# zengxiaofei/HapHiC

Measured on AMD Instinct MI355X. Metric: Hi-C pairs/s ingested (link-matrix build) + MCL iters/s, higher is better.
Workload: dtype u64 keys + u32 counts (ingest); f32 values, exact u64 fixed-point accumulation (MCL)

## Files before the change

haphic_amd/csrc/hhx_expand.hip:

```cpp
#include <chrono>
#include <climits>

#include "hhx_common.h"
#include "hhx_internal.h"
#include "hhx_sort.h"

using namespace hhx;

struct ExpandDemand { i64 out = 0, cand = 0; };
thread_local ExpandDemand g_expand_hint, g_expand_demand;
void hhx_expand_set_hint(i64 out, i64 cand) { g_expand_hint.out = out; g_expand_hint.cand = cand; }
void hhx_expand_last_demand(i64 *out, i64 *cand) { *out = g_expand_demand.out; *cand = g_expand_demand.cand; }

namespace {

constexpr int EX_T_WIN = 1024;
constexpr int EX_T_CMP = 256;
constexpr int EX_T_MAX = 1024;
constexpr int EX_WAVES_MAX = EX_T_MAX / HHX_WAVE;
#define EX_T ((int)blockDim.x)
#define EX_WAVES ((int)blockDim.x / HHX_WAVE)
constexpr int STAGE = 1024;
constexpr int MAX_WIN = 512;
constexpr int N_DUMMY = HHX_WAVE;
// ... 1522 lines not shown
            const i32 len = min(STAGE, a_e - a0);
            stage_chunk(P, l, a0, len);
            __syncthreads();
            mark_compact(P, l, len);
            __syncthreads();
        }
        const i32 nnz_row = bitmap_prefix_total(l, W);
        nnzc += (tid == 0) ? nnz_row : 0;
        double s_run = 0.0;
        i32 n_win = 0;
        for (i32 r0 = 0; r0 < nnz_row; r0 += cap, ++n_win) {
            const i32 rlen = min(cap, nnz_row - r0);
            for (i32 t = tid; t < rlen; t += EX_T) l.acc[t] = 0;
            __syncthreads();
            for (i32 a0 = a_b; a0 < a_e; a0 += STAGE) {
                const i32 len = min(STAGE, a_e - a0);
                stage_chunk(P, l, a0, len);
                __syncthreads();
                accumulate_compact(P, l, len, r0, rlen);
                __syncthreads();
            }
            i32 nz;
            s_run += window_power_sum<true>(P, l, rlen, &nz);
            window_emit_candidates<true>(P, l, rlen, 0, r0, s_run, &l.win_off[n_win], &l.win_cnt[n_win]);
            __syncthreads();
        }
        if (nnz_row == 0) {
            if (tid == 0) { P.row_off[row] = 0; P.row_cnt[row] = 0; }
        } else finalize_row(P, l, row, n_win, s_run, l.win_off, l.win_cnt);
        __syncthreads();
    }
    nnzc = wave_sum_i64(nnzc);
    if (lane_id() == 0 && nnzc) atomicAdd(&P.cursors[3], (unsigned long long)nnzc);
}

constexpr int HASH_T = 512, HASH_C = 4096, HASH_LIMIT = 3072, HASH_STAGE = 256, HASH_PER = HASH_C / HASH_T, HASH_PROBES = 128;
constexpr int HASH_U = 4;
constexpr u32 HASH_EMPTY = 0xffffffffu;
#ifdef HHX_HASH_STATS
__device__ unsigned long long g_hash_stats[4];
#endif
__host__ __device__ inline size_t hash_lds_bytes(i32 W) {
    const size_t tail = (size_t)W * 8 > (size_t)(HASH_T / HHX_WAVE) * HHX_WAVE * 8 ? (size_t)W * 8 : (size_t)(HASH_T / HHX_WAVE) * HHX_WAVE * 8;
    return (size_t)(HASH_C + HHX_WAVE) * 8 + (size_t)HASH_C * 4 + (size_t)HASH_STAGE * (8 + 4 + 4) + (size_t)EX_WAVES_MAX * (8 + 4 + 4) + 8 + (8 + 4) + 16 + tail;
}
__device__ __forceinline__ u32 hash_slot(u32 col) { return __umul24(col, 0x9e3779u) >> 20; }
__device__ __forceinline__ bool hash_try(u64 *acc, u32 *keys, i32 *ctr, u32 slot, u32 seen, u32 col, u64 g) {
    if (seen == HASH_EMPTY) {
        seen = atomicCAS(&keys[slot], HASH_EMPTY, col);
        if (seen == HASH_EMPTY) {
            if (atomicAdd(&ctr[0], 1) >= HASH_LIMIT) ctr[1] = 1;
            seen = col;
        }
    }
    if (seen != col) return false;
    atomicAdd((unsigned long long *)&acc[slot], (unsigned long long)g);
    return true;
}
__device__ __forceinline__ i32 wave_incl_scan_dpp(i32 v) {
    v += __builtin_amdgcn_update_dpp(0, v, 0x111, 0xf, 0xf, true);
    v += __builtin_amdgcn_update_dpp(0, v, 0x112, 0xf, 0xf, true);
    v += __builtin_amdgcn_update_dpp(0, v, 0x114, 0xf, 0xf, true);
    v += __builtin_amdgcn_update_dpp(0, v, 0x118, 0xf, 0xf, true);
    v += __builtin_amdgcn_update_dpp(0, v, 0x142, 0xa, 0xf, false);
    v += __builtin_amdgcn_update_dpp(0, v, 0x143, 0xc, 0xf, false);
    return v;
}
__device__ __forceinline__ void hash_insert(u64 *acc, u32 *keys, i32 *ctr, u32 col, u64 g) {
    u32 slot = hash_slot(col) & (HASH_C - 2);
    for (int probes = 0;; ++probes) {
        const uint2 c2 = *reinterpret_cast<const uint2 *>(&keys[slot]);
        if (hash_try(acc, keys, ctr, slot, c2.x, col, g) || hash_try(acc, keys, ctr, slot + 1, c2.y, col, g)) break;
        if (probes >= HASH_PROBES) { ctr[1] = 1; break; }
        slot = (slot + 2) & (HASH_C - 2);
    }
}
__device__ __forceinline__ void hash_drain(u64 *acc, u32 *keys, i32 *ctr, const int2 *__restrict__ Bjx, const double *st_da, const u64 *wq, i32 n) {
    for (i32 i = lane_id(); i < n; i += HHX_WAVE) {
        const u64 w = wq[i];
        const int2 e = Bjx[(i32)(u32)w];
        hash_insert(acc, keys, ctr, (u32)e.x, fx_bits_prod(st_da[(i32)(w >> 32)], (double)__int_as_float(e.y)));
    }
}
__device__ __forceinline__ void hash_consume(u64 *acc, u32 *keys, i32 *ctr, const int2 *__restrict__ Bjx, const double *st_da, u64 *wq, i32 wq_cap, i32 &wq_n,
                                             const int4 (&t)[HASH_U], i32 q_first, i32 qb, i32 qe, double da, i32 e_staged) {
    constexpr int K = 2 * HASH_U;
    uint2 cur[K];
#pragma unroll
    for (int k = 0; k < K; ++k) {
        const u32 col = (u32)((k & 1) ? t[k >> 1].z : t[k >> 1].x);
        cur[k] = *reinterpret_cast<const uint2 *>(&keys[hash_slot(col) & (HASH_C - 2)]);
    }
    const u32 scratch = HASH_C + (u32)lane_id();
    u32 pend = 0;
#pragma unroll
    for (int k = 0; k < K; ++k) {
        const i32 q = q_first + (k >> 1) * 2 * HHX_WAVE + (k & 1);
        const bool valid = (k & 1) ? q < qe : (q >= qb && q < qe);
        const u32 col = (u32)((k & 1) ? t[k >> 1].z : t[k >> 1].x);
        const bool m0 = cur[k].x == col, m1 = cur[k].y == col;
        const bool hit = valid && (m0 || m1);
        const u64 g = fx_bits_prod(da, (double)__int_as_float((k & 1) ? t[k >> 1].w : t[k >> 1].y));
        atomicAdd((unsigned long long *)&acc[hit ? (hash_slot(col) & (HASH_C - 2)) + (m0 ? 0u : 1u) : scratch], (unsigned long long)g);
        pend |= (valid && !hit) ? 1u << k : 0u;
    }
#ifdef HHX_HASH_STATS
    {
        const i32 c = __popc(pend);
        i32 mx = c;
#pragma unroll
        for (int o = 32; o > 0; o >>= 1) mx = max(mx, __shfl_down(mx, o, HHX_WAVE));
        const i32 sm = wave_sum_i32(c);
        if (lane_id() == 0) { atomicAdd(&g_hash_stats[0], 1ull); atomicAdd(&g_hash_stats[1], (unsigned long long)sm); atomicAdd(&g_hash_stats[2], (unsigned long long)mx); }
    }
#endif
    const i32 c = __popc(pend);
    const i32 incl = wave_incl_scan_dpp(c);
    const i32 total = __builtin_amdgcn_readlane(incl, HHX_WAVE - 1);
    if (total == 0) return;
    if (wq_n + total > wq_cap) {
        hash_drain(acc, keys, ctr, Bjx, st_da, wq, wq_n);
        wq_n = 0;
        if (total > wq_cap) {
            while (pend) {
                const int k = __ffs((int)pend) - 1;
                pend &= pend - 1;
                const int2 e = Bjx[q_first + (k >> 1) * 2 * HHX_WAVE + (k & 1)];
                hash_insert(acc, keys, ctr, (u32)e.x, fx_bits_prod(da, (double)__int_as_float(e.y)));
            }
            return;
        }
    }
    i32 at = wq_n + incl - c;
    while (pend) {
        const int k = __ffs((int)pend) - 1;
        pend &= pend - 1;
        wq[at++] = (u64)(u32)(q_first + (k >> 1) * 2 * HHX_WAVE + (k & 1)) | ((u64)(u32)e_staged << 32);
    }
    wq_n += total;
}
__global__ __launch_bounds__(256) void k_pack_jx(i64 n, const i32 *__restrict__ j, const float *__restrict__ x, int2 *__restrict__ out) {
    for (i64 k = (i64)blockIdx.x * blockDim.x + threadIdx.x; k < n; k += (i64)gridDim.x * blockDim.x) out[k] = make_int2(j[k], __float_as_int(x[k]));
}
__global__ __launch_bounds__(HASH_T, 4) void k_expand_hash(ExParams P, const i32 *__restrict__ rows, i32 n_list, i32 W, const i64 *__restrict__ row_f,
                                                        i64 window_min, i32 *__restrict__ list_window, i32 *__restrict__ list_compact,
                                                        unsigned int *__restrict__ counts) {
    extern __shared__ __attribute__((aligned(16))) unsigned char smem[];
    ExLds l;
    unsigned char *p = smem;
    l.acc = (u64 *)p; p += (size_t)(HASH_C + HHX_WAVE) * 8;
    l.st_da = (double *)p; p += HASH_STAGE * 8;
    l.red_d = (double *)p; p += EX_WAVES_MAX * 8;
    l.bcast = (i64 *)p; p += 8;
    l.win_off = (i64 *)p; p += 8;
    u32 *keys = (u32 *)p; p += (size_t)HASH_C * 4;
    l.st_qb = (i32 *)p; p += HASH_STAGE * 4;
    l.st_qe = (i32 *)p; p += HASH_STAGE * 4;
    l.red_i = (i32 *)p; p += EX_WAVES_MAX * 4;
    l.red_f = (float *)p; p += EX_WAVES_MAX * 4;
    l.win_cnt = (i32 *)p; p += 4;
    l.ctr = (i32 *)p; p += 12;
    l.bitmap = (u32 *)p; p += (size_t)W * 4;
    l.prefix = (u32 *)p;
    const int tid = threadIdx.x, lane = lane_id(), wave = tid / HHX_WAVE;
    const i32 region = max(2 * W, (HASH_T / HHX_WAVE) * HHX_WAVE * 2);
    const i32 wq_cap = ((region / 2) / (HASH_T / HHX_WAVE)) & ~(HHX_WAVE - 1);
    u64 *const wq = reinterpret_cast<u64 *>(l.bitmap) + (size_t)wave * wq_cap;
    i64 nnzc = 0;
    for (i32 li = blockIdx.x; li < n_list; li += gridDim.x) {
        const i32 row = rows[li];
        const i32 a_b = P.Ap[row], a_e = P.Ap[row + 1];
        for (i32 t = tid; t < HASH_C; t += HASH_T) { keys[t] = HASH_EMPTY; l.acc[t] = 0; }
        if (tid == 0) { l.ctr[0] = 0; l.ctr[1] = 0; }
        __syncthreads();
        bool fits = true;
        i32 wq_n = 0;
        for (i32 a0 = a_b; a0 < a_e && fits; a0 += HASH_STAGE) {
            const i32 len = min(HASH_STAGE, a_e - a0);
            stage_chunk(P, l, a0, len);
            __syncthreads();
            for (i32 e = 2 * wave; e < len; e += 2 * (HASH_T / HHX_WAVE)) {
                const bool two = e + 1 < len;
                const double da0 = l.st_da[e], da1 = two ? l.st_da[e + 1] : 0.0;
                const i32 qb0 = l.st_qb[e], qe0 = l.st_qe[e], qb1 = two ? l.st_qb[e + 1] : 0, qe1 = two ? l.st_qe[e + 1] : 0;
                const i32 s0 = qb0 & ~1, s1 = qb1 & ~1;
                const i32 span = max(qe0 - s0, qe1 - s1);
                for (i32 off = 0; off < span; off += HASH_U * 2 * HHX_WAVE) {
                    int4 t0[HASH_U], t1[HASH_U];
#pragma unroll
                    for (int u = 0; u < HASH_U; ++u) {
                        const i32 q = s0 + off + u * 2 * HHX_WAVE + 2 * lane;
                        t0[u] = *reinterpret_cast<const int4 *>(P.Bjx + (q < qe0 ? q : s0));
                    }
#pragma unroll
                    for (int u = 0; u < HASH_U; ++u) {
                        const i32 q = s1 + off + u * 2 * HHX_WAVE + 2 * lane;
                        t1[u] = *reinterpret_cast<const int4 *>(P.Bjx + (q < qe1 ? q : s1));
                    }
                    if (__hip_atomic_load(&l.ctr[1], __ATOMIC_RELAXED, __HIP_MEMORY_SCOPE_WORKGROUP)) break;
                    hash_consume(l.acc, keys, l.ctr, P.Bjx, l.st_da, wq, wq_cap, wq_n, t0, s0 + off + 2 * lane, qb0, qe0, da0, e);
                    hash_consume(l.acc, keys, l.ctr, P.Bjx, l.st_da, wq, wq_cap, wq_n, t1, s1 + off + 2 * lane, qb1, qe1, da1, e + 1);
                }
                if (__hip_atomic_load(&l.ctr[1], __ATOMIC_RELAXED, __HIP_MEMORY_SCOPE_WORKGROUP)) break;
            }
            hash_drain(l.acc, keys, l.ctr, P.Bjx, l.st_da, wq, wq_n);
            wq_n = 0;
            __syncthreads();
            fits = l.ctr[1] == 0;
            __syncthreads();
        }
        if (!fits) {
            if (tid == 0) {
                const i64 f = row_f[row];
                if (f >= window_min) {
                    list_window[atomicAdd(&counts[0], 1u)] = row;
                    atomicAdd(&P.cursors[5], (unsigned long long)f);
                    atomicAdd(&P.cursors[6], (unsigned long long)(a_e - a_b));
                } else list_compact[atomicAdd(&counts[1], 1u)] = row;
            }
            continue;
        }
        for (i32 w = tid; w < W; w += HASH_T) l.bitmap[w] = 0;
        __syncthreads();
        u32 kk[HASH_PER];
        u64 aa[HASH_PER];
#pragma unroll
        for (int u = 0; u < HASH_PER; ++u) {
            const i32 t = tid + u * HASH_T;
            kk[u] = keys[t];
            aa[u] = l.acc[t];
            if (kk[u] != HASH_EMPTY) atomicOr(&l.bitmap[kk[u] >> 5], 1u << (kk[u] & 31));
        }
        __syncthreads();
        const i32 nnz_row = bitmap_prefix_total(l, W);
#pragma unroll
        for (int u = 0; u < HASH_PER; ++u)
            if (kk[u] != HASH_EMPTY) l.acc[rank_of(l, (i32)kk[u])] = aa[u];
        __syncthreads();
        nnzc += (tid == 0) ? nnz_row : 0;
        if (nnz_row == 0) {
            if (tid == 0) { P.row_off[row] = 0; P.row_cnt[row] = 0; }
        } else {
            i32 nz;
            const double s_run = window_power_sum<true>(P, l, nnz_row, &nz);
            window_emit_candidates<true>(P, l, nnz_row, 0, 0, s_run, &l.win_off[0], &l.win_cnt[0]);
            __syncthreads();
            finalize_row(P, l, row, 1, s_run, l.win_off, l.win_cnt);
        }
        __syncthreads();
    }
    nnzc = wave_sum_i64(nnzc);
    if (lane_id() == 0 && nnzc) atomicAdd(&P.cursors[3], (unsigned long long)nnzc);
}

__global__ __launch_bounds__(256) void k_transpose_lower(float *__restrict__ Y, i64 ld, i32 n, i32 cap) {
    __shared__ float tile[64][65];
    i32 bj = 1, bi = (i32)blockIdx.z;
    while (bi >= bj) { bi -= bj; ++bj; }
    const i32 r0 = bj * cap + blockIdx.y * 64, c0 = bi * cap + blockIdx.x * 64;
    if (r0 >= n) return;
    const int tx = threadIdx.x & 63, ty = threadIdx.x >> 6;
    for (int k = ty; k < 64; k += 4) {
        const i32 sr = c0 + k, sc = r0 + tx;
        tile[k][tx] = (sr < n && sc < n) ? Y[(size_t)sr * (size_t)ld + sc] : 0.0f;
    }
    __syncthreads();
    for (int k = ty; k < 64; k += 4) {
        const i32 dr = r0 + k, dc = c0 + tx;
        if (dr < n && dc < n) Y[(size_t)dr * (size_t)ld + dc] = tile[tx][k];
    }
}

__global__ __launch_bounds__(256) void k_transpose_tri(const float *__restrict__ tri, float *__restrict__ dst, i64 dst_ld, i32 I, i32 rows_I, i32 cap, i64 ldn) {
    __shared__ float tile[64][65];
    const i32 J = (i32)blockIdx.z;
    const float *src = tri + tri_row_off(J, cap, ldn) + (size_t)(I - J) * cap;
    const i64 src_ld = ldn - (i64)J * cap;
    const i32 r0 = blockIdx.y * 64, c0 = blockIdx.x * 64;
    if (r0 >= rows_I) return;
    const int tx = threadIdx.x & 63, ty = threadIdx.x >> 6;
    for (int k = ty; k < 64; k += 4)
        tile[k][tx] = (r0 + tx < rows_I) ? src[(size_t)(c0 + k) * (size_t)src_ld + r0 + tx] : 0.0f;
    __syncthreads();
    for (int k = ty; k < 64; k += 4)
        if (r0 + k < rows_I) dst[(size_t)(r0 + k) * (size_t)dst_ld + (size_t)J * cap + c0 + tx] = tile[tx][k];
// ... 352 lines not shown
    pl.cap_g = 0; pl.n_win_g = 0;
    if (pl.reuse_R) {
        static_assert(win_fixed_bytes() == 784, "GroupStride assumes the window kernel's fixed LDS bytes");
        const i32 cols_max = (pl.reuse_R == 4 ? GroupStride<4>::value : GroupStride<2>::value) - N_DUMMY;
        for (i64 wn = std::max<i64>(1, ((i64)n_cols + cols_max - 1) / cols_max);; ++wn) {
            const i32 c = (i32)((((i64)n_cols + wn - 1) / wn + 63) & ~63);
            if (c <= cols_max) { pl.cap_g = c; pl.n_win_g = (n_cols + c - 1) / c; break; }
        }
        if (pl.cap_g < 1024) pl.reuse_R = 0;
    }
    pl.n_win_tab = std::max(pl.n_win, pl.n_win_g);
    if (pl.cap_win + N_DUMMY > 65536) return fail("expand: column window wider than 16 bits");
    return 0;
}

static void expand_pool_sizes(const ExPlan &pl, const hhx_csr *a, RowPools &tab) {
    tab.pool_cap = pl.dense ? 64 : std::max<i64>(4 * a->nnz + 16 * (i64)pl.n_rows, (i64)1 << 22);
    tab.cand_cap = pl.dense ? 64 : (pl.n_win > 1 ? 2 * tab.pool_cap : tab.pool_cap);
    if (pl.dense || pl.raw) return;
    if (g_expand_hint.out > 0) {
        tab.pool_cap = std::max<i64>(g_expand_hint.out + g_expand_hint.out / 2 + 16 * (i64)pl.n_rows, (i64)1 << 22);
        tab.cand_cap = std::max<i64>(g_expand_hint.cand + g_expand_hint.cand / 2 + 16 * (i64)pl.n_rows, (i64)1 << 22);
    }
    g_expand_hint = ExpandDemand();
}

static ExParams expand_params(const ExPlan &pl, const hhx_csr *a, const hhx_csr *b, const CodedOperand &coded, double inflation, double pruning) {
    ExParams P;
    memset(&P, 0, sizeof P);
    P.Ap = a->indptr.p; P.Aj = a->indices.p; P.Ax = a->data.p;
    P.Bp = b->indptr.p; P.Bj = b->indices.p; P.Bx = b->data.p;
    P.n_rows = pl.n_rows; P.n_cols = pl.n_cols;
    P.scale = ldexp(1.0, pl.fx_shift - 52); P.inv_scale = ldexp(1.0, 52 - pl.fx_shift);
    P.r = (double)(float)inflation; P.square = inflation == 2.0; P.thr = (float)pruning;
    P.raw = coded.raw;
    P.n_win = pl.n_win;
    P.dense = coded.dense_out; P.dense_ld = coded.dense_ld ? coded.dense_ld : (i64)pl.n_cols;
    P.W = pl.fx ? coded.W : nullptr; P.A16 = coded.a16; P.row_div = coded.a_row_sum; P.fx_inv = ldexp(1.0, -coded.shift);
    P.sym = coded.sym; P.sym_row0 = coded.sym_row0;
    P.tri = coded.tri; P.tri_ldn = (i64)pl.n_win * pl.cap_win;
    P.Sc16 = nullptr; P.Sx = nullptr; P.rec = nullptr; P.Bjx = nullptr; P.narrow_classes = 0; P.wb = WB_MAX;
    return P;
}

struct RowLists {
    DevBuf<i32> w, c, t, h;
    DevBuf<i64> row_f;
    DevBuf<unsigned int> counts;
    int alloc(i32 n_rows) {
        return w.alloc((size_t)n_rows + 1) || c.alloc((size_t)n_rows + 1) || t.alloc((size_t)n_rows + 1) || h.alloc((size_t)n_rows + 1) ||
               row_f.alloc((size_t)n_rows + 1) || counts.alloc(4);
    }
};
struct ClassCounts {
    unsigned int classified[4];
    unsigned int hc[4];
    unsigned long long hw[2];
};
static int read_class_counts(const RowLists &L, const RowPools &tab, ClassCounts &cc) {
    HHX_HIP(hipMemcpyAsync(cc.hc, L.counts.p, sizeof cc.hc, hipMemcpyDeviceToHost, g_stream));
    HHX_HIP(hipMemcpyAsync(cc.hw, tab.cursors.p + 5, sizeof cc.hw, hipMemcpyDeviceToHost, g_stream));
    HHX_HIP(hipStreamSynchronize(g_stream));
    return 0;
}
static int classify(const hhx_csr *a, const hhx_csr *b, i64 window_min, i64 hash_max, i64 tiny_max, RowLists &L, RowPools &tab, ClassCounts *cc) {
    HHX_HIP(hipMemsetAsync(L.counts.p, 0, 4 * sizeof(unsigned int), g_stream));
    HHX_TRY(tab.zero_cursors());
    k_classify<<<(unsigned)std::max<i64>(1, std::min<i64>(((i64)a->n_rows + 63) / 64, 4096)), 256, 0, g_stream>>>(
        a->n_rows, a->indptr.p, a->indices.p, b->indptr.p, window_min, hash_max, tiny_max, L.w.p, L.c.p, L.t.p, L.h.p, L.row_f.p, L.counts.p, tab.cursors.p);
    HHX_LAUNCH_CHECK();
    if (!cc) return 0;
    HHX_TRY(read_class_counts(L, tab, *cc));
    memcpy(cc->classified, cc->hc, sizeof cc->hc);
    return 0;
}

static int run_hash_class(const ExPlan &pl, const hhx_csr *b, ExParams &P, RowLists &L, const RowPools &tab, DevBuf<int2> &bjx, ClassCounts &cc) {
    if (!bjx.p) {
        if (bjx.alloc((size_t)b->nnz + 4)) return 1;
        k_pack_jx<<<(unsigned)std::max<i64>(1, std::min<i64>((b->nnz + 255) / 256, 256 * 16)), 256, 0, g_stream>>>(b->nnz, b->indices.p, b->data.p, bjx.p);
        HHX_LAUNCH_CHECK();
    }
    P.Bjx = bjx.p;
    HHX_TRY((raise_dynamic_lds<k_expand_hash>()));
    {
        KTimer kt("expand_hash");
        const unsigned per_cu = pl.lds_hash > 80 * 1024 ? 1 : 2;
        k_expand_hash<<<std::min<unsigned>(cc.hc[3], 256 * per_cu * 4), HASH_T, pl.lds_hash, g_stream>>>(P, L.h.p, (i32)cc.hc[3], pl.W, L.row_f.p, pl.window_min,
                                                                                                     L.w.p, L.c.p, L.counts.p);
#ifdef HHX_HASH_STATS
        {
            unsigned long long hs[4] = {0, 0, 0, 0};
            (void)hipStreamSynchronize(g_stream);
            (void)hipMemcpyFromSymbol(hs, HIP_SYMBOL(g_hash_stats), sizeof hs);
            fprintf(stderr, "[hash stats] rows %u: consumes %llu, leftovers %llu (%.2f per consume of 512), sum of per-consume maxima %llu (%.2f per consume)\n", cc.hc[3], hs[0], hs[1],
                    hs[0] ? (double)hs[1] / hs[0] : 0.0, hs[2], hs[0] ? (double)hs[2] / hs[0] : 0.0);
            unsigned long long z[4] = {0, 0, 0, 0};
            (void)hipMemcpyToSymbol(HIP_SYMBOL(g_hash_stats), z, sizeof z);
        }
#endif
    }
    HHX_LAUNCH_CHECK();
    return read_class_counts(L, tab, cc);
}

struct KeyedRows {
    DevBuf<u64> key, val, skey, sval;
    int alloc(i64 nl) { return key.alloc((size_t)nl) || val.alloc((size_t)nl) || skey.alloc((size_t)nl) || sval.alloc((size_t)nl); }
    int sort(i64 nl, i32 n_rows, int key_bits) {
        int rbits = 1;
        while (rbits < 31 && (n_rows >> rbits)) ++rbits;
        HHX_TRY(stable_sort_pairs_u64(val.p, sval.p, key.p, skey.p, nl, rbits));
        HHX_TRY(stable_sort_pairs_u64(skey.p, key.p, sval.p, val.p, nl, key_bits));
        return 0;
    }
};

struct RowGroups {
    DevBuf<i32> rows, Gp, Gj;
    DevBuf<float> Gx;
    i32 n = 0;
    i64 entries = 0;
    bool on = false;
};
static int build_groups(const ExPlan &pl, const hhx_csr *a, const RowLists &L, const ClassCounts &cc, RowGroups &g) {
    g.on = false;
    g.n = 0;
    const int R = pl.reuse_R;
    const double a_len0 = cc.hc[0] ? (double)cc.hw[1] / (double)cc.hc[0] : 0.0;
    if (!R || cc.hc[0] < 1024 || a_len0 < 128.0) return 0;
    KTimer kt("group_build");
    const i64 nl = (i64)cc.hc[0];
    KeyedRows kr;
    if (kr.alloc(nl)) return 1;
    k_row_attractor<<<(unsigned)std::min<i64>((nl + 3) / 4, 4096), 256, 0, g_stream>>>((i32)nl, L.w.p, a->indptr.p, a->indices.p, a->data.p, kr.key.p, kr.val.p);
    HHX_LAUNCH_CHECK();
    int cbits = 1;
    while (cbits < 31 && (pl.n_cols >> cbits)) ++cbits;
    HHX_TRY(kr.sort(nl, pl.n_rows, cbits));
    std::vector<u64> h_att((size_t)nl), h_row((size_t)nl);
    HHX_HIP(hipMemcpyAsync(h_att.data(), kr.key.p, 8 * (size_t)nl, hipMemcpyDeviceToHost, g_stream));
    HHX_HIP(hipMemcpyAsync(h_row.data(), kr.val.p, 8 * (size_t)nl, hipMemcpyDeviceToHost, g_stream));
    HHX_HIP(hipStreamSynchronize(g_stream));
    std::vector<i32> h_grp;
    h_grp.reserve((size_t)nl + (size_t)R);
    for (i64 p0 = 0; p0 < nl;) {
        i64 p1 = p0 + 1;
        while (p1 < nl && p1 - p0 < R && h_att[(size_t)p1] == h_att[(size_t)p0]) ++p1;
        for (i64 q = p0; q < p0 + R; ++q) h_grp.push_back(q < p1 ? (i32)h_row[(size_t)q] : -1);
        p0 = p1;
    }
    g.n = (i32)(h_grp.size() / (size_t)R);
    if ((i64)g.n * 2 > nl) return 0;
    const i32 Wb = (pl.n_cols + 31) / 32;
    const size_t lds_u = (size_t)Wb * 8 + 64;
    DevBuf<i32> gcnt;
    if (g.rows.alloc(h_grp.size()) || gcnt.alloc((size_t)g.n + 1) || g.Gp.alloc((size_t)g.n + 2)) return 1;
    HHX_HIP(hipMemcpyAsync(g.rows.p, h_grp.data(), sizeof(i32) * h_grp.size(), hipMemcpyHostToDevice, g_stream));
    HHX_TRY((raise_dynamic_lds<k_group_union<false>, k_group_union<true>>()));
    if (lds_u > 160 * 1024) return 0;
    const unsigned ggrid = (unsigned)std::min<i32>(g.n, 256 * 8);
    k_group_union<false><<<ggrid, 256, lds_u, g_stream>>>(g.n, R, g.rows.p, a->indptr.p, a->indices.p, a->data.p, Wb, gcnt.p, nullptr, nullptr, nullptr);
    HHX_LAUNCH_CHECK();
    i64 union_nnz = 0;
    HHX_TRY(exclusive_scan_i32(gcnt.p, g.Gp.p, g.n, &union_nnz));
    if (union_nnz >= (i64)INT32_MAX / 8) return 0;
    if (g.Gj.alloc((size_t)union_nnz + 1) || g.Gx.alloc((size_t)union_nnz * (size_t)R + 1)) return 1;
    k_group_union<true><<<ggrid, 256, lds_u, g_stream>>>(g.n, R, g.rows.p, a->indptr.p, a->indices.p, a->data.p, Wb, nullptr, g.Gp.p, g.Gj.p, g.Gx.p);
    HHX_LAUNCH_CHECK();
    HHX_HIP(hipStreamSynchronize(g_stream));
    g.on = true;
    g.entries = union_nnz;
// ... 578 lines not shown
```

haphic_amd/csrc/hhx_runtime.hip:

```cpp
#include <chrono>

#include "hhx_common.h"
#include "hhx_internal.h"

namespace hhx {

thread_local std::string g_err;
thread_local hipStream_t g_stream = nullptr;

thread_local Arena *g_arena = nullptr;

namespace {
std::mutex g_pool_mu;
std::multimap<size_t, void *> g_free;
struct Live { size_t size; Arena *owner; };
std::map<void *, Live> g_live;
std::vector<void *> g_quarantine;
std::map<void *, int> g_prewarmed;

size_t size_class(size_t bytes) {
    size_t c = 256;
    while (c < bytes) {
        if (c >= (size_t(64) << 20)) return (bytes + (size_t(64) << 20) - 1) / (size_t(64) << 20) * (size_t(64) << 20);
        c <<= 1;
// ... 250 lines not shown
    HHX_LAUNCH_CHECK();
    if (total_host) {
        T t;
        HHX_HIP(hipMemcpyAsync(&t, out + n, sizeof(T), hipMemcpyDeviceToHost, g_stream));
        HHX_HIP(hipStreamSynchronize(g_stream));
        *total_host = (i64)t;
    }
    return 0;
}

void u64_copy_async(const unsigned long long *src, unsigned long long *dst, i64 n) {
    (void)hipMemcpyAsync(dst, src, sizeof(unsigned long long) * (size_t)n, hipMemcpyDeviceToDevice, g_stream);
}

__global__ __launch_bounds__(256) void k_sum_i32_wide(const i32 *__restrict__ in, i64 n, unsigned long long *__restrict__ total) {
    i64 s = 0;
    for (i64 i = (i64)blockIdx.x * blockDim.x + threadIdx.x; i < n; i += (i64)gridDim.x * blockDim.x) s += in[i];
    s = wave_sum_i64(s);
    if (lane_id() == 0 && s) atomicAdd(total, (unsigned long long)s);
}
int exclusive_scan_i32(const i32 *in, i32 *out, i64 n, i64 *total_host) {
    if (n > 0) {
        DevBuf<unsigned long long> wide;
        if (wide.alloc(1)) return 1;
        HHX_HIP(hipMemsetAsync(wide.p, 0, sizeof(unsigned long long), g_stream));
        k_sum_i32_wide<<<(unsigned)std::max<i64>(1, std::min<i64>((n + 255) / 256, 1024)), 256, 0, g_stream>>>(in, n, wide.p);
        HHX_LAUNCH_CHECK();
        unsigned long long t = 0;
        HHX_HIP(hipMemcpyAsync(&t, wide.p, sizeof t, hipMemcpyDeviceToHost, g_stream));
        HHX_HIP(hipStreamSynchronize(g_stream));
        if (t > (unsigned long long)INT32_MAX)
            return fail("a matrix of %llu entries exceeds the int32 index range of hhx_csr (scipy's too): split the operand into row blocks "
                        "(hhx_csr_row_block) or use the fused iteration (hhx_expand_inflate_prune)", t);
    }
    return scan_total<i32>(in, out, n, total_host);
}
int exclusive_scan_i64(const i64 *in, i64 *out, i64 n, i64 *total_host) { return scan_total<i64>(in, out, n, total_host); }

}

using namespace hhx;

extern "C" const char *hhx_last_error(void) { return g_err.c_str(); }
extern "C" int hhx_version(void) { return 100; }
extern "C" int hhx_device_count(int *count) {
    HHX_HIP(hipGetDeviceCount(count));
    return 0;
}
extern "C" int hhx_set_device(int device) {
    HHX_HIP(hipSetDevice(device));
    return 0;
}
extern "C" int hhx_set_stream(void *s) {
    if ((hipStream_t)s != g_stream) HHX_HIP(hipDeviceSynchronize());
    g_stream = (hipStream_t)s;
    return 0;
}
extern "C" int hhx_synchronize(void) {
    HHX_HIP(hipStreamSynchronize(g_stream));
    return 0;
}
extern "C" int hhx_pool_prewarm(int32_t n, const int64_t *bytes) {
    if (n < 0 || (n && !bytes)) return fail("hhx_pool_prewarm: bad argument");
    for (i32 k = 0; k < n; ++k) {
        if (bytes[k] <= 0) continue;
        void *p = nullptr;
        if (hipMalloc(&p, size_class((size_t)bytes[k])) != hipSuccess) { (void)hipGetLastError(); break; }
        std::lock_guard<std::mutex> lk(g_pool_mu);
        g_free.emplace(size_class((size_t)bytes[k]), p);
        g_prewarmed[p] = 0;
    }
    return 0;
}

extern "C" int hhx_pool_trim(void) {
    pool_trim(false);
    return 0;
}
extern "C" int hhx_pool_trim_keep(int64_t keep_bytes) {
    if (keep_bytes < 0) return fail("hhx_pool_trim_keep: bad argument");
    pool_trim(false, keep_bytes);
    return 0;
}
static const char *const k_tune_names[] = {"cls", "cls_nc", "cls_balance", "links_integer", "links_sym", "hash_max", "tile_u", "win_batch",
                                           "cache_slice_mb", "dense_tri", "reuse", "row_order", "dense_seed_hint", "block_tiles", "correct_agg",
                                           "plotnorm_small", "plotnorm_chunk_cells", "sort_lds_shape", "groupstats_lds_slots", "reassign_window",
#ifdef HHX_PROBE_BUILD
                                           "probe",
#endif
                                           nullptr};
extern "C" int hhx_tune(const char *name, int64_t value) {
    if (!name) return fail("null name");
    bool known = false;
    for (const char *const *k = k_tune_names; *k; ++k) known |= strcmp(*k, name) == 0;
    if (!known) return fail("hhx_tune: unknown knob '%s'", name);
    std::lock_guard<std::mutex> lk(g_tune_mu);
    if (value == INT64_MIN) g_tune.erase(name);
    else g_tune[name] = value;
    return 0;
}
extern "C" int hhx_profile_enable(int on) {
    g_prof_on = on != 0;
    return 0;
}
extern "C" int hhx_profile_reset(void) {
    prof_collect();
    std::lock_guard<std::mutex> lk(g_prof_mu);
    g_prof_total.clear();
    g_prof_counters.clear();
    return 0;
}
extern "C" int hhx_profile_counter(const char *name, i64 *value) {
    if (!name || !value) return fail("null pointer");
    std::lock_guard<std::mutex> lk(g_prof_mu);
    auto it = g_prof_counters.find(name);
    *value = it == g_prof_counters.end() ? 0 : it->second;
    return 0;
}
extern "C" int hhx_profile_get(const char *kernel, double *total_ms, i64 *launches) {
    if (!kernel) return fail("null kernel name");
    prof_collect();
    std::lock_guard<std::mutex> lk(g_prof_mu);
    auto it = g_prof_total.find(kernel);
    if (total_ms) *total_ms = it == g_prof_total.end() ? 0.0 : it->second.first;
    if (launches) *launches = it == g_prof_total.end() ? 0 : it->second.second;
    return 0;
}

static int csr_alloc(i32 n_rows, i32 n_cols, i64 nnz, hhx_csr **out) {
    if (n_rows < 0 || n_cols < 0 || nnz < 0) return fail("negative matrix dimension");
    if (nnz > INT32_MAX) return fail("nnz %lld exceeds the int32 index range of scipy CSC", (long long)nnz);
    hhx_csr *m = new hhx_csr();
    m->n_rows = n_rows; m->n_cols = n_cols; m->nnz = nnz;
    if (m->indptr.alloc((size_t)n_rows + 1) || m->indices.alloc((size_t)nnz) || m->data.alloc((size_t)nnz)) {
        delete m;
        return 1;
    }
    *out = m;
    return 0;
}
int hhx_csr_alloc_internal(i32 n_rows, i32 n_cols, i64 nnz, hhx_csr **out) { return csr_alloc(n_rows, n_cols, nnz, out); }

extern "C" int hhx_csr_from_host(i32 n_rows, i32 n_cols, const i32 *indptr, const i32 *indices, const float *data,
                                 hhx_csr **out) {
    if (!indptr || !out) return fail("hhx_csr_from_host: null pointer");
    i64 nnz = indptr[n_rows];
    hhx_csr *m = nullptr;
    HHX_TRY(csr_alloc(n_rows, n_cols, nnz, &m));
    hipError_t e = hipMemcpyAsync(m->indptr.p, indptr, sizeof(i32) * ((size_t)n_rows + 1), hipMemcpyHostToDevice, g_stream);
    if (e == hipSuccess && nnz) e = hipMemcpyAsync(m->indices.p, indices, sizeof(i32) * (size_t)nnz, hipMemcpyHostToDevice, g_stream);
    if (e == hipSuccess && nnz) e = hipMemcpyAsync(m->data.p, data, sizeof(float) * (size_t)nnz, hipMemcpyHostToDevice, g_stream);
    if (e == hipSuccess) e = hipStreamSynchronize(g_stream);
    if (e != hipSuccess) { delete m; return fail("hhx_csr_from_host: copy failed: %s", hipGetErrorString(e)); }
    *out = m;
    return 0;
}

extern "C" int hhx_csr_from_device(i32 n_rows, i32 n_cols, i64 nnz, const i32 *indptr, const i32 *indices,
                                   const float *data, hhx_csr **out) {
    hhx_csr *m = nullptr;
    HHX_TRY(csr_alloc(n_rows, n_cols, nnz, &m));
    hipError_t e = hipMemcpyAsync(m->indptr.p, indptr, sizeof(i32) * ((size_t)n_rows + 1), hipMemcpyDeviceToDevice, g_stream);
    if (e == hipSuccess && nnz) e = hipMemcpyAsync(m->indices.p, indices, sizeof(i32) * (size_t)nnz, hipMemcpyDeviceToDevice, g_stream);
    if (e == hipSuccess && nnz) e = hipMemcpyAsync(m->data.p, data, sizeof(float) * (size_t)nnz, hipMemcpyDeviceToDevice, g_stream);
    if (e != hipSuccess) { delete m; return fail("hhx_csr_from_device: copy failed: %s", hipGetErrorString(e)); }
    *out = m;
    return 0;
// ... 153 lines not shown
```

Before: 17.55 billion.

## Pack short B rows into whole-wave octets in hash expand kernel

```diff
diff --git a/haphic_amd/csrc/hhx_expand.hip b/haphic_amd/csrc/hhx_expand.hip
--- a/haphic_amd/csrc/hhx_expand.hip
+++ b/haphic_amd/csrc/hhx_expand.hip
@@ -1628,8 +1628,10 @@
         hash_insert(acc, keys, ctr, (u32)e.x, fx_bits_prod(st_da[(i32)(w >> 32)], (double)__int_as_float(e.y)));
     }
 }
-__device__ __forceinline__ void hash_consume(u64 *acc, u32 *keys, i32 *ctr, const int2 *__restrict__ Bjx, const double *st_da, u64 *wq, i32 wq_cap, i32 &wq_n,
-                                             const int4 (&t)[HASH_U], i32 q_first, i32 qb, i32 qe, double da, i32 e_staged) {
+struct HashRow { i32 q_first, qb, qe; double da; };
+template <bool NARROW>
+__device__ __forceinline__ void hash_consume(u64 *acc, u32 *keys, i32 *ctr, const int2 *__restrict__ Bjx, const double *st_da, const i32 *st_qb, u64 *wq, i32 wq_cap,
+                                             i32 &wq_n, const int4 (&t)[HASH_U], const HashRow (&row)[NARROW ? HASH_U : 1], i32 e_staged) {
     constexpr int K = 2 * HASH_U;
     uint2 cur[K];
 #pragma unroll
@@ -1641,12 +1643,13 @@
     u32 pend = 0;
 #pragma unroll
     for (int k = 0; k < K; ++k) {
-        const i32 q = q_first + (k >> 1) * 2 * HHX_WAVE + (k & 1);
-        const bool valid = (k & 1) ? q < qe : (q >= qb && q < qe);
+        const HashRow &r = row[NARROW ? k >> 1 : 0];
+        const i32 q = r.q_first + (NARROW ? 0 : (k >> 1) * 2 * HHX_WAVE) + (k & 1);
+        const bool valid = (k & 1) ? q < r.qe : (q >= r.qb && q < r.qe);
         const u32 col = (u32)((k & 1) ? t[k >> 1].z : t[k >> 1].x);
         const bool m0 = cur[k].x == col, m1 = cur[k].y == col;
         const bool hit = valid && (m0 || m1);
-        const u64 g = fx_bits_prod(da, (double)__int_as_float((k & 1) ? t[k >> 1].w : t[k >> 1].y));
+        const u64 g = fx_bits_prod(r.da, (double)__int_as_float((k & 1) ? t[k >> 1].w : t[k >> 1].y));
         atomicAdd((unsigned long long *)&acc[hit ? (hash_slot(col) & (HASH_C - 2)) + (m0 ? 0u : 1u) : scratch], (unsigned long long)g);
         pend |= (valid && !hit) ? 1u << k : 0u;
     }
@@ -1671,23 +1674,123 @@
             while (pend) {
                 const int k = __ffs((int)pend) - 1;
                 pend &= pend - 1;
-                const int2 e = Bjx[q_first + (k >> 1) * 2 * HHX_WAVE + (k & 1)];
-                hash_insert(acc, keys, ctr, (u32)e.x, fx_bits_prod(da, (double)__int_as_float(e.y)));
+                if constexpr (NARROW) {
+                    const i32 es = e_staged + (k >> 1);
+                    const int2 e = Bjx[(st_qb[es] & ~1) + 2 * lane_id() + (k & 1)];
+                    hash_insert(acc, keys, ctr, (u32)e.x, fx_bits_prod(st_da[es], (double)__int_as_float(e.y)));
+                } else {
+                    const int2 e = Bjx[row[0].q_first + (k >> 1) * 2 * HHX_WAVE + (k & 1)];
+                    hash_insert(acc, keys, ctr, (u32)e.x, fx_bits_prod(row[0].da, (double)__int_as_float(e.y)));
+                }
             }
             return;
         }
     }
     i32 at = wq_n + incl - c;
-    while (pend) {
-        const int k = __ffs((int)pend) - 1;
-        pend &= pend - 1;
-        wq[at++] = (u64)(u32)(q_first + (k >> 1) * 2 * HHX_WAVE + (k & 1)) | ((u64)(u32)e_staged << 32);
+    if constexpr (NARROW) {
+#pragma unroll
+        for (int k = 0; k < K; ++k)
+            if (pend & (1u << k)) wq[at++] = (u64)(u32)(row[k >> 1].q_first + (k & 1)) | ((u64)(u32)(e_staged + (k >> 1)) << 32);
+    } else {
+        while (pend) {
+            const int k = __ffs((int)pend) - 1;
+            pend &= pend - 1;
+            wq[at++] = (u64)(u32)(row[0].q_first + (k >> 1) * 2 * HHX_WAVE + (k & 1)) | ((u64)(u32)e_staged << 32);
+        }
     }
     wq_n += total;
 }
 __global__ __launch_bounds__(256) void k_pack_jx(i64 n, const i32 *__restrict__ j, const float *__restrict__ x, int2 *__restrict__ out) {
     for (i64 k = (i64)blockIdx.x * blockDim.x + threadIdx.x; k < n; k += (i64)gridDim.x * blockDim.x) out[k] = make_int2(j[k], __float_as_int(x[k]));
 }
+__device__ __forceinline__ void hash_walk_pair(const ExParams &P, const ExLds &l, u32 *keys, u64 *wq, i32 wq_cap, i32 &wq_n, i32 e, i32 len) {
+    const int lane = lane_id();
+    const bool two = e + 1 < len;
+    const double da0 = l.st_da[e], da1 = two ? l.st_da[e + 1] : 0.0;
+    const i32 qb0 = l.st_qb[e], qe0 = l.st_qe[e], qb1 = two ? l.st_qb[e + 1] : 0, qe1 = two ? l.st_qe[e + 1] : 0;
+    const i32 s0 = qb0 & ~1, s1 = qb1 & ~1;
+    const i32 span = max(qe0 - s0, qe1 - s1);
+    for (i32 off = 0; off < span; off += HASH_U * 2 * HHX_WAVE) {
+        int4 t0[HASH_U], t1[HASH_U];
+#pragma unroll
+        for (int u = 0; u < HASH_U; ++u) {
+            const i32 q = s0 + off + u * 2 * HHX_WAVE + 2 * lane;
+            t0[u] = *reinterpret_cast<const int4 *>(P.Bjx + (q < qe0 ? q : s0));
+        }
+#pragma unroll
+        for (int u = 0; u < HASH_U; ++u) {
+            const i32 q = s1 + off + u * 2 * HHX_WAVE + 2 * lane;
+            t1[u] = *reinterpret_cast<const int4 *>(P.Bjx + (q < qe1 ? q : s1));
+        }
+        if (__hip_atomic_load(&l.ctr[1], __ATOMIC_RELAXED, __HIP_MEMORY_SCOPE_WORKGROUP)) break;
+        const HashRow r0[1] = {{s0 + off + 2 * lane, qb0, qe0, da0}}, r1[1] = {{s1 + off + 2 * lane, qb1, qe1, da1}};
+        hash_consume<false>(l.acc, keys, l.ctr, P.Bjx, l.st_da, l.st_qb, wq, wq_cap, wq_n, t0, r0, e);
+        hash_consume<false>(l.acc, keys, l.ctr, P.Bjx, l.st_da, l.st_qb, wq, wq_cap, wq_n, t1, r1, e + 1);
+    }
+}
+constexpr int HASH_NARROW = 2 * HHX_WAVE;
+__device__ __forceinline__ i32 lane_value(i32 v, int j) { return __builtin_amdgcn_readlane(v, j); }
+__device__ __forceinline__ void hash_walk_narrow(const ExParams &P, const ExLds &l, u32 *keys, u64 *wq, i32 wq_cap, i32 &wq_n, i32 e0, i32 cnt) {
+    const int lane = lane_id();
+    const bool have = lane < cnt;
+    const i32 v_qb = have ? l.st_qb[e0 + lane] : 0, v_qe = have ? l.st_qe[e0 + lane] : 0;
+    const double v_da = have ? l.st_da[e0 + lane] : 0.0;
+    const i32 v_lo = __double2loint(v_da), v_hi = __double2hiint(v_da);
+    int4 t[2][HASH_U];
+#pragma unroll
+    for (int j = 0; j < 2 * HASH_U; ++j) {
+        const i32 qb = lane_value(v_qb, j), qe = lane_value(v_qe, j);
+        const i32 q = (qb & ~1) + 2 * lane;
+        t[j / HASH_U][j % HASH_U] = *reinterpret_cast<const int4 *>(P.Bjx + (q < qe ? q : (qb & ~1)));
+    }
+    if (__hip_atomic_load(&l.ctr[1], __ATOMIC_RELAXED, __HIP_MEMORY_SCOPE_WORKGROUP)) return;
+#pragma unroll
+    for (int g = 0; g < 2; ++g) {
+        HashRow r[HASH_U];
+#pragma unroll
+        for (int u = 0; u < HASH_U; ++u) {
+            const int j = g * HASH_U + u;
+            const i32 qb = lane_value(v_qb, j);
+            r[u] = {(qb & ~1) + 2 * lane, qb, lane_value(v_qe, j), __hiloint2double(lane_value(v_hi, j), lane_value(v_lo, j))};
+        }
+        hash_consume<true>(l.acc, keys, l.ctr, P.Bjx, l.st_da, l.st_qb, wq, wq_cap, wq_n, t[g], r, e0 + g * HASH_U);
+    }
+}
+__device__ __forceinline__ i32 hash_stage_sorted(const ExParams &P, const ExLds &l, i32 a0, i32 len) {
+    static_assert(HASH_STAGE <= HASH_T && HASH_STAGE % HHX_WAVE == 0, "one staged entry per thread");
+    constexpr int SW = HASH_STAGE / HHX_WAVE;
+    const int tid = threadIdx.x, wave = tid / HHX_WAVE;
+    const bool have = tid < len;
+    double da = 0.0;
+    i32 qb = 0, qe = 0;
+    if (have) {
+        const i32 k = P.Aj[a0 + tid];
+        da = (double)P.Ax[a0 + tid] * P.scale;
+        qb = P.Bp[k];
+        qe = P.Bp[k + 1];
+    }
+    const bool narrow = have && qe - (qb & ~1) <= HASH_NARROW;
+    const u64 vote = __ballot(narrow);
+    if (lane_id() == 0 && wave < SW) l.red_i[wave] = __popcll(vote);
+    __syncthreads();
+    i32 n_narrow = 0, before = 0;
+#pragma unroll
+    for (int w = 0; w < SW; ++w) {
+        const i32 c = l.red_i[w];
+        n_narrow += c;
+        before += w < wave ? c : 0;
+    }
+    if (have) {
+        before += (i32)__builtin_amdgcn_mbcnt_hi((u32)(vote >> 32), __builtin_amdgcn_mbcnt_lo((u32)vote, 0u));
+        const i32 at = narrow ? before : n_narrow + (tid - before);
+        l.st_da[at] = da;
+        l.st_qb[at] = qb;
+        l.st_qe[at] = qe;
+    }
+    __syncthreads();
+    return n_narrow;
+}
+template <bool NARROW>
 __global__ __launch_bounds__(HASH_T, 4) void k_expand_hash(ExParams P, const i32 *__restrict__ rows, i32 n_list, i32 W, const i64 *__restrict__ row_f,
                                                         i64 window_min, i32 *__restrict__ list_window, i32 *__restrict__ list_compact,
                                                         unsigned int *__restrict__ counts) {
@@ -1708,7 +1811,7 @@
     l.ctr = (i32 *)p; p += 12;
     l.bitmap = (u32 *)p; p += (size_t)W * 4;
     l.prefix = (u32 *)p;
-    const int tid = threadIdx.x, lane = lane_id(), wave = tid / HHX_WAVE;
+    const int tid = threadIdx.x, wave = tid / HHX_WAVE;
     const i32 region = max(2 * W, (HASH_T / HHX_WAVE) * HHX_WAVE * 2);
     const i32 wq_cap = ((region / 2) / (HASH_T / HHX_WAVE)) & ~(HHX_WAVE - 1);
     u64 *const wq = reinterpret_cast<u64 *>(l.bitmap) + (size_t)wave * wq_cap;
@@ -1723,30 +1826,23 @@
         i32 wq_n = 0;
         for (i32 a0 = a_b; a0 < a_e && fits; a0 += HASH_STAGE) {
             const i32 len = min(HASH_STAGE, a_e - a0);
-            stage_chunk(P, l, a0, len);
-            __syncthreads();
-            for (i32 e = 2 * wave; e < len; e += 2 * (HASH_T / HHX_WAVE)) {
-                const bool two = e + 1 < len;
-                const double da0 = l.st_da[e], da1 = two ? l.st_da[e + 1] : 0.0;
-                const i32 qb0 = l.st_qb[e], qe0 = l.st_qe[e], qb1 = two ? l.st_qb[e + 1] : 0, qe1 = two ? l.st_qe[e + 1] : 0;
-                const i32 s0 = qb0 & ~1, s1 = qb1 & ~1;
-                const i32 span = max(qe0 - s0, qe1 - s1);
-                for (i32 off = 0; off < span; off += HASH_U * 2 * HHX_WAVE) {
-                    int4 t0[HASH_U], t1[HASH_U];
-#pragma unroll
-                    for (int u = 0; u < HASH_U; ++u) {
-                        const i32 q = s0 + off + u * 2 * HHX_WAVE + 2 * lane;
-                        t0[u] = *reinterpret_cast<const int4 *>(P.Bjx + (q < qe0 ? q : s0));
-                    }
-#pragma unroll
-                    for (int u = 0; u < HASH_U; ++u) {
-                        const i32 q = s1 + off + u * 2 * HHX_WAVE + 2 * lane;
-                        t1[u] = *reinterpret_cast<const int4 *>(P.Bjx + (q < qe1 ? q : s1));
-                    }
+            constexpr int WAVES = HASH_T / HHX_WAVE;
+            i32 long_b = 0, long_w = wave;
+            if constexpr (NARROW) {
+                const i32 n_narrow = __builtin_amdgcn_readfirstlane(hash_stage_sorted(P, l, a0, len));
+                const i32 n_oct = (n_narrow + 2 * HASH_U - 1) / (2 * HASH_U);
+                for (i32 o = __builtin_amdgcn_readfirstlane(wave); o < n_oct; o += WAVES) {
+                    hash_walk_narrow(P, l, keys, wq, wq_cap, wq_n, o * 2 * HASH_U, min(2 * HASH_U, n_narrow - o * 2 * HASH_U));
                     if (__hip_atomic_load(&l.ctr[1], __ATOMIC_RELAXED, __HIP_MEMORY_SCOPE_WORKGROUP)) break;
-                    hash_consume(l.acc, keys, l.ctr, P.Bjx, l.st_da, wq, wq_cap, wq_n, t0, s0 + off + 2 * lane, qb0, qe0, da0, e);
-                    hash_consume(l.acc, keys, l.ctr, P.Bjx, l.st_da, wq, wq_cap, wq_n, t1, s1 + off + 2 * lane, qb1, qe1, da1, e + 1);
                 }
+                long_b = n_narrow;
+                long_w = (wave - n_oct) & (WAVES - 1);
+            } else {
+                stage_chunk(P, l, a0, len);
+                __syncthreads();
+            }
+            for (i32 e = long_b + 2 * long_w; e < len; e += 2 * WAVES) {
+                hash_walk_pair(P, l, keys, wq, wq_cap, wq_n, e, len);
                 if (__hip_atomic_load(&l.ctr[1], __ATOMIC_RELAXED, __HIP_MEMORY_SCOPE_WORKGROUP)) break;
             }
             hash_drain(l.acc, keys, l.ctr, P.Bjx, l.st_da, wq, wq_n);
@@ -2265,12 +2361,13 @@
         HHX_LAUNCH_CHECK();
     }
     P.Bjx = bjx.p;
-    HHX_TRY((raise_dynamic_lds<k_expand_hash>()));
+    HHX_TRY((raise_dynamic_lds<k_expand_hash<true>, k_expand_hash<false>>()));
     {
         KTimer kt("expand_hash");
         const unsigned per_cu = pl.lds_hash > 80 * 1024 ? 1 : 2;
-        k_expand_hash<<<std::min<unsigned>(cc.hc[3], 256 * per_cu * 4), HASH_T, pl.lds_hash, g_stream>>>(P, L.h.p, (i32)cc.hc[3], pl.W, L.row_f.p, pl.window_min,
-                                                                                                     L.w.p, L.c.p, L.counts.p);
+        const auto kernel = tune_get("hash_narrow", 1) ? k_expand_hash<true> : k_expand_hash<false>;
+        kernel<<<std::min<unsigned>(cc.hc[3], 256 * per_cu * 4), HASH_T, pl.lds_hash, g_stream>>>(P, L.h.p, (i32)cc.hc[3], pl.W, L.row_f.p, pl.window_min, L.w.p, L.c.p,
+                                                                                              L.counts.p);
 #ifdef HHX_HASH_STATS
         {
             unsigned long long hs[4] = {0, 0, 0, 0};
diff --git a/haphic_amd/csrc/hhx_runtime.hip b/haphic_amd/csrc/hhx_runtime.hip
--- a/haphic_amd/csrc/hhx_runtime.hip
+++ b/haphic_amd/csrc/hhx_runtime.hip
@@ -356,7 +356,7 @@
     pool_trim(false, keep_bytes);
     return 0;
 }
-static const char *const k_tune_names[] = {"cls", "cls_nc", "cls_balance", "links_integer", "links_sym", "hash_max", "tile_u", "win_batch",
+static const char *const k_tune_names[] = {"cls", "cls_nc", "cls_balance", "links_integer", "links_sym", "hash_max", "hash_narrow", "tile_u", "win_batch",
                                            "cache_slice_mb", "dense_tri", "reuse", "row_order", "dense_seed_hint", "block_tiles", "correct_agg",
                                            "plotnorm_small", "plotnorm_chunk_cells", "sort_lds_shape", "groupstats_lds_slots", "reassign_window",
 #ifdef HHX_PROBE_BUILD
```

New measurement: 17.25 billion. 0.983x the previous value.
